# burn-research/OpenMEASURE

Measured on AMD Instinct MI355X. Metric: SPR fit+reconstruct throughput (GB/s snapshot matrix), higher is better.
Workload: dtype f64

## Files before the change

### include/spr_hip.h

```cpp
#ifndef SPR_HIP_H
#define SPR_HIP_H

#include <stddef.h>
#include <stdint.h>

#ifdef __cplusplus
extern "C" {
#endif

#define SPR_OK 0
#define SPR_E_INVALID (-1)
#define SPR_E_UNSUPPORTED (-2)
#define SPR_E_HIP (-3)
#define SPR_E_WORKSPACE (-4)

#define SPR_MAX_M 256
#define SPR_MAX_M_WIDE 512
#define SPR_MAX_R 128
#define SPR_MAX_R_STREAM 256
#define SPR_MAX_R_WIDE 1024

#define SPR_ABI_VERSION 5
int spr_abi_version(void);
const char *spr_last_error(void);
// ... 68 lines not shown
int spr_project_stream_norms_f64(const double *d_X, int64_t n_rows, int32_t m, int64_t ldx, int64_t row0,
                                 int64_t n_points, int32_t n_features, int32_t center, const double *d_inv_scale,
                                 const double *d_rowmean, const double *d_W, int32_t r, double *d_Ur, int64_t ldu,
                                 double *d_rownorm2, void *d_workspace, size_t workspace_bytes, void *stream);

int spr_scale_rows_f64(const double *d_X, int64_t n_rows, int32_t m, int64_t ldx, int64_t row0,
                       int64_t n_points, int32_t n_features, const double *d_rowmean,
                       const double *d_inv_scale, double *d_X0, int64_t ldo, void *stream);
int spr_unscale_f64(const double *d_x0, int64_t n_rows, int64_t row0, int64_t n_points,
                    int32_t n_features, const double *d_rowmean, const double *d_scale,
                    const double *d_rowscale, double *d_x, void *stream);

size_t spr_feature_minmax_workspace(int32_t n_features);
int spr_feature_minmax_f64(const double *d_X, int64_t n_rows, int32_t m, int64_t ldx, int64_t row0,
                           int64_t n_points, int32_t n_features, double *d_minmax,
                           void *d_workspace, size_t workspace_bytes, void *stream);

int spr_feature_digit_hist_f64(const double *d_X, int64_t n_rows, int32_t m, int64_t ldx, int64_t row0,
                               int64_t n_points, int32_t n_features, const uint64_t *d_prefix, int32_t shift,
                               int32_t bits, int32_t two_targets, uint64_t *d_hist, void *stream);

size_t spr_colsums_workspace(int32_t m, int32_t n_features);
int spr_colsums_f64(const double *d_X, int64_t n_rows, int32_t m, int64_t ldx, int64_t row0,
                    int64_t n_points, int32_t n_features, const double *d_rowmean, double *d_out,
                    void *d_workspace, size_t workspace_bytes, void *stream);
int spr_fill_feature_f64(double *d_out, int64_t n_rows, int64_t row0, int64_t n_points, int32_t n_features,
                         const double *d_values, void *stream);

int spr_reconstruct_f64(const double *d_Ur, int64_t n_rows, int32_t r, int64_t ldu,
                        int64_t row0, int64_t n_points, int32_t n_features,
                        const double *d_rowmean, const double *d_scale, const double *d_rowscale,
                        const double *d_A, int32_t n_p, double *d_Xrec, int64_t ldo,
                        void *stream);
size_t spr_bound_sweep_workspace(int32_t n_p, int32_t n_features);
int spr_bound_sweep_f64(const double *d_Ur, int64_t n_rows, int32_t r, int64_t ldu, int64_t row0, int64_t n_points,
                        int32_t n_features, const double *d_rowmean, const double *d_scale, const double *d_limits,
                        const double *d_clamp, const double *d_G, int32_t n_p, double tol, int32_t k, double *d_out,
                        void *d_workspace, size_t workspace_bytes, void *stream);
int spr_bound_sweep_u32(const float *d_Ur, int64_t n_rows, int32_t r, int64_t ldu, int64_t row0, int64_t n_points,
                        int32_t n_features, const double *d_rowmean, const double *d_scale, const double *d_limits,
                        const double *d_clamp, const double *d_G, int32_t n_p, double tol, int32_t k, double *d_out,
                        void *d_workspace, size_t workspace_bytes, void *stream);
size_t spr_bound_sweep_batch_workspace(int32_t n_p, int32_t n_features);
int spr_bound_sweep_batch_f64(const double *d_Ur, int64_t n_rows, int32_t r, int64_t ldu, int64_t row0, int64_t n_points,
                              int32_t n_features, const double *d_rowmean, const double *d_scale, const double *d_limits,
                              const double *d_clamp, const double *d_G, int32_t n_p, double tol, int32_t k, double *d_out,
                              void *d_workspace, size_t workspace_bytes, void *stream);
int spr_bound_sweep_batch_u32(const float *d_Ur, int64_t n_rows, int32_t r, int64_t ldu, int64_t row0, int64_t n_points,
                              int32_t n_features, const double *d_rowmean, const double *d_scale, const double *d_limits,
                              const double *d_clamp, const double *d_G, int32_t n_p, double tol, int32_t k, double *d_out,
                              void *d_workspace, size_t workspace_bytes, void *stream);
size_t spr_encode_workspace(int32_t r, int32_t k, int32_t n_features);
int spr_encode_f64(const double *d_Ur, int64_t n_rows, int32_t r, int64_t ldu, const double *d_X, int32_t k, int64_t ldx,
                   int64_t row0, int64_t n_points, int32_t n_features, const double *d_rowmean, const double *d_scale,
                   double *d_A, void *d_workspace, size_t workspace_bytes, void *stream);
int spr_encode_x32(const double *d_Ur, int64_t n_rows, int32_t r, int64_t ldu, const float *d_X, int32_t k, int64_t ldx,
                   int64_t row0, int64_t n_points, int32_t n_features, const double *d_rowmean, const double *d_scale,
                   double *d_A, void *d_workspace, size_t workspace_bytes, void *stream);
int spr_encode_u32(const float *d_Ur, int64_t n_rows, int32_t r, int64_t ldu, const double *d_X, int32_t k, int64_t ldx,
                   int64_t row0, int64_t n_points, int32_t n_features, const double *d_rowmean, const double *d_scale,
                   double *d_A, void *d_workspace, size_t workspace_bytes, void *stream);
int spr_encode_x32_u32(const float *d_Ur, int64_t n_rows, int32_t r, int64_t ldu, const float *d_X, int32_t k, int64_t ldx,
                       int64_t row0, int64_t n_points, int32_t n_features, const double *d_rowmean, const double *d_scale,
                       double *d_A, void *d_workspace, size_t workspace_bytes, void *stream);
size_t spr_field_error_workspace(int32_t k, int32_t n_features);
int spr_field_error_f64(const double *d_Ur, int64_t n_rows, int32_t r, int64_t ldu, int64_t row0, int64_t n_points,
// ... 311 lines not shown
```

### openmeasure_amd/_lib.py

```python
from __future__ import annotations

import ctypes as C
import os

_HERE = os.path.dirname(os.path.abspath(__file__))
LIB_PATH = os.environ.get('SPR_HIP_LIBRARY') or os.path.join(_HERE, 'libspr_hip.so')

SPR_ABI_VERSION = 5
SPR_MAX_M = 256
SPR_MAX_M_WIDE = 512
SPR_MAX_R = 128
SPR_MAX_R_STREAM = 256
SPR_MAX_R_WIDE = 1024
SPR_GP_MAX_M = 800
SPR_GP_MAX_D = 8

_i32, _i64, _u64, _sz = C.c_int32, C.c_int64, C.c_uint64, C.c_size_t
_p = C.c_void_p
_dbl = C.c_double

PROTOTYPES = {
    'spr_abi_version': (C.c_int, []),
    'spr_last_error': (C.c_char_p, []),
    'spr_device_cus': (C.c_int, [C.POINTER(C.c_int)]),
# ... 1 lines not shown
    'spr_download_bytes': (C.c_int, [_p, _p, _i64, _p, _u64, _p]),
    'spr_host_tridiag_vectors': (C.c_int, [_p, _p, _i32, _p, _i32, _p, _i32]),
    'spr_host_eig_top': (C.c_int, [_p, _i32, _i32, _p, _p, _p, _p, _p]),
    'spr_host_svd_top': (C.c_int, [_p, _i32, _i32, _p, _p, _p, _p, _p]),
    'spr_stats_gram_workspace': (_sz, [_i32, _i32]),
    'spr_stats_gram_f64': (C.c_int, [_p, _i64, _i32, _i64, _i64, _i64, _i32, _i32, _p, _p, _sz, _p]),
    'spr_stats_gram_finalize_f64': (C.c_int, [_i64, _i32, _i64, _i64, _i32, _p, _sz, _p, _p, _i32, _i32, _p]),
    'spr_stats_gram_shifted_f64': (C.c_int, [_p, _i64, _i32, _i64, _i64, _i64, _i32, _p, _p, _p, _sz, _p]),
    'spr_gram_shift_finish_f64': (C.c_int, [_p, _p, _i64, _i32, _i32, _p, _i32, _p]),
    'spr_rowstats_workspace': (_sz, [_i32]),
    'spr_rowstats_f64': (C.c_int, [_p, _i64, _i32, _i64, _i64, _i64, _i32, _p, _p, _p, _sz, _p]),
    'spr_gram_cross_workspace': (_sz, [_i32, _i32]),
    'spr_gram_cross_f64': (C.c_int, [_p, _i64, _i32, _i64, _i64, _i64, _i32, _i32, _p, _p, _p, _sz, _p]),
    'spr_gram_cross_pair_f64': (C.c_int, [_p, _i64, _i32, _i32, _i32, _i32, _i64, _i64, _i64, _i32, _i32, _p, _p, _p, _sz, _p]),
    'spr_rowmean_stats_f64': (C.c_int, [_p, _i64, _i64, _i64, _i32, _p, _p, _sz, _p]),
    'spr_spectrum_max_m': (_i32, []),
    'spr_spectrum_f64': (C.c_int, [_p, _p, _i32, _i32, _i32, _i32, _i32, _p, _p, _p, _p, _p, _p, _p, _p, _p, _p, _p]),
    'spr_gram_combine_f64': (C.c_int, [_p, _p, _i32, _i32, _i32, _i32, _p, _p, _p, _p, _p]),
    'spr_project_f64': (C.c_int, [_p, _i64, _i32, _i64, _i64, _i64, _i32, _i32, _p, _p, _p, _i32, _p, _i64, _i32, _p]),
    'spr_project_norms_supported': (_i32, [_i32, _i32, _i64, _i64, _p, _i32]),
    'spr_project_norms_f64': (C.c_int, [_p, _i64, _i32, _i64, _i64, _i64, _i32, _i32, _p, _p, _p, _i32, _p, _i64, _p, _p]),
    'spr_project_stream_norms_f64': (C.c_int, [_p, _i64, _i32, _i64, _i64, _i64, _i32, _i32, _p, _p, _p, _i32, _p, _i64, _p, _p, _sz, _p]),
    'spr_project_stream_workspace': (_sz, [_i32, _i32, _i32]),
    'spr_project_stream_f64': (C.c_int, [_p, _i64, _i32, _i64, _i64, _i64, _i32, _i32, _p, _p, _p, _i32, _p, _i64, _p, _sz, _p]),
    'spr_scale_rows_f64': (C.c_int, [_p, _i64, _i32, _i64, _i64, _i64, _i32, _p, _p, _p, _i64, _p]),
    'spr_unscale_f64': (C.c_int, [_p, _i64, _i64, _i64, _i32, _p, _p, _p, _p, _p]),
    'spr_feature_minmax_workspace': (_sz, [_i32]),
    'spr_feature_minmax_f64': (C.c_int, [_p, _i64, _i32, _i64, _i64, _i64, _i32, _p, _p, _sz, _p]),
    'spr_feature_digit_hist_f64': (C.c_int, [_p, _i64, _i32, _i64, _i64, _i64, _i32, _p, _i32, _i32, _i32, _p, _p]),
    'spr_colsums_workspace': (_sz, [_i32, _i32]),
    'spr_colsums_f64': (C.c_int, [_p, _i64, _i32, _i64, _i64, _i64, _i32, _p, _p, _p, _sz, _p]),
    'spr_fill_feature_f64': (C.c_int, [_p, _i64, _i64, _i64, _i32, _p, _p]),
    'spr_reconstruct_f64': (C.c_int, [_p, _i64, _i32, _i64, _i64, _i64, _i32, _p, _p, _p, _p, _i32, _p, _i64, _p]),
    'spr_bound_sweep_workspace': (_sz, [_i32, _i32]),
    'spr_bound_sweep_f64': (C.c_int, [_p, _i64, _i32, _i64, _i64, _i64, _i32, _p, _p, _p, _p, _p, _i32, _dbl, _i32, _p, _p, _sz, _p]),
    'spr_bound_sweep_batch_workspace': (_sz, [_i32, _i32]),
    'spr_bound_sweep_batch_f64': (C.c_int, [_p, _i64, _i32, _i64, _i64, _i64, _i32, _p, _p, _p, _p, _p, _i32, _dbl, _i32, _p, _p, _sz, _p]),
    'spr_encode_workspace': (_sz, [_i32, _i32, _i32]),
    'spr_encode_f64': (C.c_int, [_p, _i64, _i32, _i64, _p, _i32, _i64, _i64, _i64, _i32, _p, _p, _p, _p, _sz, _p]),
    'spr_field_error_workspace': (_sz, [_i32, _i32]),
    'spr_field_error_f64': (C.c_int, [_p, _i64, _i32, _i64, _i64, _i64, _i32, _p, _p, _p, _i32, _p, _i64, _p, _p, _sz, _p]),
    'spr_gappy_normal_workspace': (_sz, [_i32, _i32, _i32]),
    'spr_gappy_normal_f64': (C.c_int, [_p, _i64, _i32, _i64, _p, _i32, _i64, _i64, _i64, _i32, _p, _p, _p, _i64, _p, _p, _p, _p, _sz, _p]),
    'spr_gappy_fill_workspace': (_sz, []),
    'spr_gappy_rowfill_f64': (C.c_int, [_p, _i64, _i32, _i64, _i64, _p, _i64, _p, _p, _sz, _p]),
    'spr_gappy_fill_f64': (C.c_int, [_p, _i64, _i32, _i64, _p, _i32, _i64, _i64, _i64, _i32, _p, _p, _p, _p, _i64, _p, _p, _sz, _p]),
    'spr_field_std_diag_f64': (C.c_int, [_p, _i64, _i32, _i64, _i64, _i64, _i32, _p, _p, _p, _i32, _p, _i64, _p]),
    'spr_field_std_factor_f64': (C.c_int, [_p, _i64, _i32, _i64, _i64, _i64, _i32, _p, _p, _p, _i32, _i32, _p, _i64, _p]),
    'spr_gp_workspace': (_sz, [_i32, _i32]),
    'spr_gp_train_f64': (C.c_int, [_p, _i32, _i32, _i64, _p, _i32, _i64, _i32, _p, _dbl, _i32, _dbl, _p, _p, _p, _p, _p, _sz, _p]),
    'spr_gp_predict_f64': (C.c_int, [_p, _i32, _i32, _i64, _p, _i32, _i64, _i32, _p, _i32, _p, _p, _p, _p, _p]),
    'spr_gp_workspace_ard': (_sz, [_i32, _i32, _i32]),
    'spr_gp_train_ard_f64': (C.c_int, [_p, _i32, _i32, _i64, _p, _i32, _i64, _i32, _i32, _p, _dbl, _i32, _dbl, _p, _p, _p, _p, _p, _sz, _p]),
    'spr_gp_predict_ard_f64': (C.c_int, [_p, _i32, _i32, _i64, _p, _i32, _i64, _i32, _i32, _p, _i32, _p, _p, _p, _p, _p]),
    'spr_field_unstage_f64': (C.c_int, [_p, _i32, _i32, _i64, _p, _i64, _p]),
    'spr_field_unstage_blocks_f64': (C.c_int, [_p, _i32, _i32, _i64, _p, _p, _i64, _p]),
    'spr_p2p_handle_bytes': (_sz, []),
    'spr_p2p_alloc': (C.c_int, [_sz, _i32, _p, _p]),
    'spr_p2p_free': (C.c_int, [_p]),
    'spr_p2p_open': (C.c_int, [_p, _p]),
    'spr_p2p_close': (C.c_int, [_p]),
    'spr_p2p_device_id': (C.c_int, [_p, _i32]),
    'spr_p2p_peer_access': (C.c_int, [_p, _p]),
    'spr_p2p_signal': (C.c_int, [_p, _u64, _p]),
    'spr_p2p_wait': (C.c_int, [_p, _u64, _p]),
    'spr_p2p_flags_set': (C.c_int, [_p, _i32, _u64, _p]),
# ... 36 lines not shown
    'spr_allreduce_f64': (C.c_int, [_p, _p, _i64, _p]),
    'spr_allreduce_i64': (C.c_int, [_p, _p, _i64, _p]),
    'spr_allgather': (C.c_int, [_p, _p, _p, _i64, _p]),
    'spr_fit_gram_pass_buffer': (_sz, [_i32, _i32, _i32]),
    'spr_fit_gram_pass_workspace': (_sz, [_i32, _i32, _i64]),
    'spr_fit_gram_pass': (C.c_int, [_p, _p, _i32, _i64, _i32, _i64, _i64, _i64, _i32, _i32, _p, _p, _sz, _p, _p, _p, _p, _p, _sz, _p]),
    'spr_synth_f64': (C.c_int, [_p, _i64, _i32, _i64, _i64, _i64, _i32, _p, _i32, _i32, _dbl, _u64, _p]),
    'spr_synth_gather_f64': (C.c_int, [_p, _i32, _i64, _i32, _p, _i32, _i32, _dbl, _u64, _p, _p]),
}

_lib = None


class SprError(RuntimeError):
    """A libspr_hip.so call returned a negative status."""


PROTOTYPES['spr_project_x32_acc'] = (C.c_int, [_p, _i64, _i32, _i64, _i64, _i64, _i32, _i32, _p, _p, _p, _i32, _p, _i64, _p, _i64, _p])

for _f64, _x32 in (('spr_stats_gram_f64', 'spr_stats_gram_x32'), ('spr_stats_gram_shifted_f64', 'spr_stats_gram_shifted_x32'), ('spr_rowstats_f64', 'spr_rowstats_x32'),
                   ('spr_gram_cross_f64', 'spr_gram_cross_x32'), ('spr_gram_cross_pair_f64', 'spr_gram_cross_pair_x32'), ('spr_project_f64', 'spr_project_x32'),
                   ('spr_project_f64', 'spr_project_x32_f64out'),
                   ('spr_project_stream_f64', 'spr_project_stream_x32'),
                   ('spr_project_stream_f64', 'spr_project_stream_x32_f64out'),
                   ('spr_project_norms_f64', 'spr_project_norms_x32'),
                   ('spr_project_norms_f64', 'spr_project_norms_x32_f64out'),
                   ('spr_project_stream_norms_f64', 'spr_project_stream_norms_x32'),
                   ('spr_project_stream_norms_f64', 'spr_project_stream_norms_x32_f64out'),
                   ('spr_qr_init_norms_f64', 'spr_qr_init_norms_u32'),
                   ('spr_qr_epoch_sweep_f64', 'spr_qr_epoch_sweep_u32'),
                   ('spr_scale_rows_f64', 'spr_scale_rows_x32'), ('spr_feature_minmax_f64', 'spr_feature_minmax_x32'),
                   ('spr_colsums_f64', 'spr_colsums_x32'), ('spr_feature_digit_hist_f64', 'spr_feature_digit_hist_x32'),
                   ('spr_synth_f64', 'spr_synth_f32'), ('spr_reconstruct_f64', 'spr_reconstruct_u32'),
                   ('spr_bound_sweep_f64', 'spr_bound_sweep_u32'),
                   ('spr_bound_sweep_batch_f64', 'spr_bound_sweep_batch_u32'),
                   ('spr_encode_f64', 'spr_encode_x32'), ('spr_encode_f64', 'spr_encode_u32'),
                   ('spr_encode_f64', 'spr_encode_x32_u32'),
                   ('spr_field_error_f64', 'spr_field_error_x32'), ('spr_field_error_f64', 'spr_field_error_u32'),
                   ('spr_field_error_f64', 'spr_field_error_x32_u32'),
                   ('spr_gappy_normal_f64', 'spr_gappy_normal_x32'), ('spr_gappy_normal_f64', 'spr_gappy_normal_u32'),
                   ('spr_gappy_normal_f64', 'spr_gappy_normal_x32_u32'),
                   ('spr_gappy_rowfill_f64', 'spr_gappy_rowfill_x32'),
                   ('spr_gappy_fill_f64', 'spr_gappy_fill_x32'), ('spr_gappy_fill_f64', 'spr_gappy_fill_u32'),
                   ('spr_gappy_fill_f64', 'spr_gappy_fill_x32_u32'),
                   ('spr_field_std_diag_f64', 'spr_field_std_diag_u32'),
                   ('spr_field_std_factor_f64', 'spr_field_std_factor_u32'),
                   ('spr_mask_rows_f64', 'spr_mask_rows_u32'), ('spr_qr_init_f64', 'spr_qr_init_u32'),
                   ('spr_qr_refresh_f64', 'spr_qr_refresh_u32'), ('spr_measure_csr_f64', 'spr_measure_csr_u32')):
    PROTOTYPES[_x32] = PROTOTYPES[_f64]


def load():
    global _lib
    if _lib is not None:
        return _lib
    if not os.path.exists(LIB_PATH):
        raise RuntimeError(
            f'{LIB_PATH} is missing: build it with `make -C openmeasure_amd/csrc` '
            '(or __graft_entry__.build()). There is no CPU fallback for the SPR kernels.')
    import torch
    lib = C.CDLL(LIB_PATH, mode=C.RTLD_GLOBAL)
    for name, (res, args) in PROTOTYPES.items():
        fn = getattr(lib, name)
        fn.restype = res
        fn.argtypes = args
    have = lib.spr_abi_version()
# ... 14 lines not shown
```

### openmeasure_amd/_shard.py

```python
from __future__ import annotations

import numpy as np

class RowShard:

    def __init__(self, row0, n_global, group=None, force_collectives=False, broadcast_basis=False, partial=False,
                 gather='auto', native_comm=False):
        if gather not in ('auto', 'p2p', 'rccl'):
            raise ValueError("gather must be 'auto', 'p2p' or 'rccl'")
        self.native_comm = bool(native_comm)
        self.row0 = int(row0)
        self.n_global = int(n_global)
        self.group = group
        self.force_collectives = bool(force_collectives)
        self.broadcast_basis = bool(broadcast_basis)
        self.partial = bool(partial)
        self.gather = gather

    @property
    def world(self):
        import torch.distributed as dist
        return dist.get_world_size(self.group) if dist.is_available() and dist.is_initialized() else 1

    @property
    def rank(self):
        import torch.distributed as dist
        return dist.get_rank(self.group) if dist.is_available() and dist.is_initialized() else 0


class PendingField:

    def __init__(self, tensor, works=(), keep=(), on_wait=None, join=None, needs_cus=True, launch=None, shape=None):
        self._tensor = tensor
        self._works = list(works)
        self._join = join
        self._keep = keep
        self._on_wait = on_wait
        self._launch = launch
        self._inner = None
        self._shape = tuple(shape) if shape is not None else None
        self._needs_cus = bool(needs_cus)

    @property
    def needs_cus(self):
        if self._inner is not None:
            return self._inner.needs_cus
        return self._needs_cus and (bool(self._works) or self._join is not None)

    @property
    def shape(self):
        return self._shape if self._tensor is None else tuple(self._tensor.shape)

    @property
    def launched(self):
        return self._launch is None

    @property
    def pending(self):
        if self._launch is not None:
            return True
        if self._inner is not None:
            return self._inner.pending
        return bool(self._works) or self._join is not None

    def launch(self):
        fn, self._launch = self._launch, None
        if fn is not None:
            res = fn()
            if isinstance(res, PendingField):
                self._inner = res
            else:
                self._tensor = res

    def wait(self):
        self.launch()
        if self._inner is not None:
            self._tensor = self._inner.wait()
            self._inner = None
            return self._tensor
        done = self._on_wait() if ((self._works or self._join is not None) and self._on_wait is not None) else None
        for w in self._works:
            w.wait()
        if self._join is not None:
            self._join()
        if done is not None:
            done()
        self._works = []
        self._join = None
        self._keep = ()
        self._on_wait = None
        return self._tensor


class ShardedOps:

    def _world(self):
        return self._shard.world if self._shard is not None else 1

    def _dist(self):
        return self._shard is not None and (self._shard.world > 1 or self._shard.force_collectives)

    def _shard_layout(self, n_loc):
        lay = self.__dict__.get('_layout')
        if lay is None:
            eng = self._engine()
            src = self.__dict__.pop('_layout_src', None)
            if src is not None:
                rows = np.rint(eng.to_host(src[0].sum(1))).astype(np.int64)
# ... 398 lines not shown
```

### openmeasure_amd/csrc/reconstruct.hip

```cpp
#include <stdlib.h>

#include <type_traits>

#include "rowtile.hpp"
#include "launch.hpp"

#ifndef SPR_RECONSTRUCT_VALU
#define SPR_RECONSTRUCT_VALU 0
#endif

namespace {

constexpr int RM_THREADS = 256;
constexpr int RM_PB = 16;

template <int MTR, int VEC, typename TU>
__global__ __launch_bounds__(RM_THREADS) void reconstruct_mfma_kernel(
    const TU *__restrict__ Ur, int r, int64_t ldu, SegPlan plan, const double *__restrict__ rowmean,
    const double *__restrict__ scale, const double *__restrict__ rowscale, const double *__restrict__ A, int64_t lda,
    int np0, int npb, double *__restrict__ out, int64_t ldo, int accumulate) {
  constexpr int NW = RM_THREADS / 64, R = 64;
  constexpr int MPAD = 16 * MTR, MP = MPAD + 2, KSTEPS = MPAD / 4;
  using RT = RowTile<MTR, R, MP, NW, 16, TU>;
  __shared__ double smem[2 * R * MP];
// ... 276 lines not shown
  SPR_REQUIRE_LAYOUT(name, row0, n_rows, n_points, n_features);
  hipStream_t st = static_cast<hipStream_t>(stream);
  if (!std::is_same<TU, double>::value || !SPR_RECONSTRUCT_VALU || r > SPR_MAX_R)
    return reconstruct_groups<TU>(d_Ur, n_rows, r, ldu, row0, n_points, n_features, d_rowmean, d_scale, d_rowscale, d_A, n_p,
                                  d_Xrec, ldo, st);
  if constexpr (std::is_same<TU, double>::value) {
    const int half = (r + 1) / 2;
#define RC(L) return launch<L>(d_Ur, n_rows, r, ldu, row0, n_points, n_features, d_rowmean, d_scale, d_rowscale, d_A, n_p, d_Xrec, ldo, st)
    if (half <= 1) RC(1);
    if (half <= 2) RC(2);
    if (half <= 4) RC(4);
    if (half <= 8) RC(8);
    if (half <= 16) RC(16);
    if (half <= 32) RC(32);
    RC(64);
#undef RC
  }
  return SPR_E_UNSUPPORTED;
}
}

#define SPR_RECONSTRUCT_ENTRY(NAME, TU)                                                                                       \
  SPR_ENTRY(NAME,                                                                                                             \
            (const TU *d_Ur, int64_t n_rows, int32_t r, int64_t ldu, int64_t row0, int64_t n_points, int32_t n_features,      \
             const double *d_rowmean, const double *d_scale, const double *d_rowscale, const double *d_A, int32_t n_p,        \
             double *d_Xrec, int64_t ldo, void *stream),                                                                      \
            (reconstruct<TU>), d_Ur, n_rows, r, ldu, row0, n_points, n_features, d_rowmean, d_scale, d_rowscale, d_A, n_p,    \
            d_Xrec, ldo, stream)
SPR_RECONSTRUCT_ENTRY(spr_reconstruct_f64, double)
SPR_RECONSTRUCT_ENTRY(spr_reconstruct_u32, float)
#undef SPR_RECONSTRUCT_ENTRY

namespace {
__global__ __launch_bounds__(256) void field_unstage_kernel(const double *__restrict__ stage, int world, int n_p,
                                                            int64_t n_loc, double *__restrict__ out, int64_t ldo) {
  const int q = blockIdx.y / n_p, v = blockIdx.y - q * n_p;
  const double *src = stage + ((int64_t)q * n_p + v) * n_loc;
  double *dst = out + (int64_t)v * ldo + (int64_t)q * n_loc;
  const bool vec = ((reinterpret_cast<uintptr_t>(src) | reinterpret_cast<uintptr_t>(dst)) & 15) == 0;
  const int64_t stride = (int64_t)gridDim.x * 256;
  if (vec) {
    const int64_t n2 = n_loc / 2;
    for (int64_t i = (int64_t)blockIdx.x * 256 + threadIdx.x; i < n2; i += stride)
      reinterpret_cast<f64x2 *>(dst)[i] = __builtin_nontemporal_load(reinterpret_cast<const f64x2 *>(src) + i);
    if ((n_loc & 1) && blockIdx.x == 0 && threadIdx.x == 0) dst[n_loc - 1] = src[n_loc - 1];
  } else {
    for (int64_t i = (int64_t)blockIdx.x * 256 + threadIdx.x; i < n_loc; i += stride) dst[i] = src[i];
  }
}
}

extern "C" int spr_field_unstage_f64(const double *d_stage, int32_t world, int32_t n_p, int64_t n_loc, double *d_out,
                                     int64_t ldo, void *stream) {
  SPR_REQUIRE(d_stage && d_out, SPR_E_INVALID, "spr_field_unstage_f64: NULL pointer");
  SPR_REQUIRE(world > 0 && n_p > 0 && n_loc > 0 && ldo >= (int64_t)world * n_loc && (int64_t)world * n_p <= 65535,
              SPR_E_INVALID, "spr_field_unstage_f64: bad shape world=%d n_p=%d n_loc=%lld ldo=%lld", world, n_p,
              (long long)n_loc, (long long)ldo);
  int64_t bx = (n_loc / 2 + 255) / 256;
  if (bx > 1024) bx = 1024;
  if (bx < 1) bx = 1;
  hipLaunchKernelGGL(field_unstage_kernel, dim3((unsigned)bx, (unsigned)(world * n_p)), dim3(256), 0,
                     static_cast<hipStream_t>(stream), d_stage, (int)world, (int)n_p, n_loc, d_out, ldo);
  SPR_LAUNCH_CHECK();
  return SPR_OK;
}

// ... 36 lines not shown
```

### openmeasure_amd/engine.py

```python
from __future__ import annotations

import numpy as np

from . import _lib


def _ptr(t):
    return t.data_ptr() if t is not None else None


_NP_OF = {'torch.float64': np.float64, 'torch.float32': np.float32, 'torch.int64': np.int64, 'torch.int32': np.int32,
          'torch.uint8': np.uint8, 'torch.int8': np.int8, 'torch.int16': np.int16, 'torch.bool': np.bool_}


class HipEngine:
    name = 'hip-gfx950'

    supports_row_norms = True
    supports_gram_out = True

    def __init__(self, device=None):
        import torch
        self.torch = torch
        if not torch.cuda.is_available():
            raise RuntimeError('openmeasure_amd needs an AMD GPU visible to PyTorch-ROCm; '
                               'there is no CPU fallback for the SPR kernels.')
        self.lib = _lib.load()
        self.device = torch.device(device if device is not None else f'cuda:{torch.cuda.current_device()}')
        self._ws = {}
        self._timing = {}
        import os
        self._force_stream = os.environ.get('SPR_PROJECT_STREAM') == '1'
        self._dl_kernel = os.environ.get('SPR_DL_KERNEL', '1') != '0'
        self._stage = None
        import atexit
        import weakref
        ref = weakref.ref(self)
        atexit.register(lambda: ref() is not None and ref().close(wait=False))

    def close(self, wait=True):
        torch = self.torch
        if wait:
            try:
                torch.cuda.synchronize(self.device)
            except RuntimeError:
                pass
        pool = self.__dict__.pop('_copy_pool', None)
        if pool is not None:
            pool.shutdown(wait=wait, cancel_futures=not wait)
        self._stage = None
        for k in ('_dstage2', '_dstage_slots', '_dl', '_reuse', '_side'):
            self.__dict__.pop(k, None)
        try:
            torch._C._host_emptyCache()
        except (AttributeError, RuntimeError):
            pass

    def _stream(self):
        return self.torch.cuda.current_stream(self.device).cuda_stream

    def empty(self, shape, dtype=None):
        return self.torch.empty(shape, dtype=dtype or self.torch.float64, device=self.device)

    def zeros(self, shape, dtype=None):
        return self.torch.zeros(shape, dtype=dtype or self.torch.float64, device=self.device)

    _STAGE_BYTES = 1 << 20
    _STAGE_SLOTS = 8

    def to_device(self, a, dtype=None):
        torch = self.torch
        if dtype is None:
            dtype = torch.float64
        t = torch.as_tensor(np.ascontiguousarray(a))
        if t.dtype != dtype:
            t = t.to(dtype)
        nbytes = t.numel() * t.element_size()
        if nbytes == 0 or nbytes > self._STAGE_BYTES or nbytes % 8:
            return t.to(device=self.device).contiguous()
        if self._stage is None:
            self._stage = [[torch.empty(self._STAGE_BYTES, dtype=torch.uint8, pin_memory=True), None]
                           for _ in range(self._STAGE_SLOTS)]
            self._stage_next = 0
        slot = self._stage[self._stage_next]
# ... 614 lines not shown
                   _ptr(ws), ws.numel(), self._stream())
        return out

    def fill_feature(self, n_rows, row0, n_points, values):
        out = self.empty((n_rows,))
        self._call(self.lib.spr_fill_feature_f64, _ptr(out), n_rows, row0, n_points, values.shape[0], _ptr(values),
                   self._stream())
        return out

    def scale_rows(self, X, row0, n_points, n_features, rowmean, inv_scale):
        n, m, ld = self._check_matrix(X)
        out = self.empty((n, m))
        self._call(self._x('spr_scale_rows', X), _ptr(X), n, m, ld, row0, n_points, n_features, _ptr(rowmean),
                   _ptr(inv_scale), _ptr(out), m, self._stream())
        return out

    def unscale(self, x0, row0, n_points, n_features, rowmean, scale, rowscale=None):
        n = x0.shape[0]
        out = self.empty((n,))
        self._call(self.lib.spr_unscale_f64, _ptr(x0.contiguous()), n, row0, n_points, n_features, _ptr(rowmean),
                   _ptr(scale), _ptr(rowscale), _ptr(out), self._stream())
        return out

    def reconstruct(self, Ur, row0, n_points, n_features, rowmean, scale, A, out=None, rowscale=None):
        n, r, ldu = self._check_matrix(Ur)
        n_p = A.shape[0]
        if out is None:
            out = self.empty((n_p, n))
        self._call(self._u('spr_reconstruct', Ur), _ptr(Ur), n, r, ldu, row0, n_points, n_features, _ptr(rowmean),
                   _ptr(scale), _ptr(rowscale), _ptr(A.contiguous()), n_p, _ptr(out), out.stride(0), self._stream(),
                   timed='reconstruct')
        return out

    def bound_sweep(self, Ur, row0, n_points, n_features, rowmean, scale, limits, clamp, G, tol, k):
        n, r, ldu = self._check_matrix(Ur)
        n_p = G.shape[0]
        out = self.empty((n_p, 3 + 3 * k))
        ws = self._workspace('bound_sweep', self.lib.spr_bound_sweep_workspace(n_p, n_features))
        self._call(self._u('spr_bound_sweep', Ur), _ptr(Ur), n, r, ldu, row0, n_points, n_features, _ptr(rowmean),
                   _ptr(scale), _ptr(limits.contiguous()), _ptr(clamp.contiguous()), _ptr(G.contiguous()), n_p, float(tol),
                   int(k), _ptr(out), _ptr(ws), ws.numel(), self._stream(), timed='bound_sweep')
        return out

    def bound_sweep_batch(self, Ur, row0, n_points, n_features, rowmean, scale, limits, clamp, G, tol, k):
        n, r, ldu = self._check_matrix(Ur)
        n_p = G.shape[0]
        out = self.empty((n_p, 3 + 3 * k))
        ws = self._workspace('bound_sweep', self.lib.spr_bound_sweep_batch_workspace(n_p, n_features))
        self._call(self._u('spr_bound_sweep_batch', Ur), _ptr(Ur), n, r, ldu, row0, n_points, n_features, _ptr(rowmean),
                   _ptr(scale), _ptr(limits.contiguous()), _ptr(clamp.contiguous()), _ptr(G.contiguous()), n_p, float(tol),
                   int(k), _ptr(out), _ptr(ws), ws.numel(), self._stream(), timed='bound_sweep_batch')
        return out

    def _ux(self, base, Ur, X):
        t = self.torch
        x32, u32 = X.dtype == t.float32, Ur.dtype == t.float32
        return getattr(self.lib, base + ('_x32_u32' if x32 and u32 else '_x32' if x32 else '_u32' if u32 else '_f64'))

    def _check_columns(self, Ur, X):
        n, r, ldu = self._check_matrix(Ur)
        if isinstance(X, self.torch.Tensor) and X.dim() == 2 and X.shape[1] == 1 and X.stride(1) != 1:
            X = X.as_strided(X.shape, (X.stride(0), 1))
        nx, k, ldx = self._check_matrix(X)
        if nx != n:
            raise ValueError(f'the matrix has {nx} rows, the basis block {n}')
        return X, n, r, ldu, k, ldx
# ... 407 lines not shown
```

### openmeasure_amd/rom.py

```python
from __future__ import annotations

from collections import namedtuple

import numpy as np

from . import _eigen
from ._lib import SPR_MAX_R, SPR_MAX_R_WIDE
from ._placement import GemPlacement, _check_mask, pivot_loop
from ._shard import PendingField, RowShard, ShardedOps

__all__ = ['ROM', 'SPR', 'RowShard', 'DeviceMatrix', 'PendingField', 'OneHotRows']

_DEVICE_SPECTRUM_MAX_M = 24
_GRAM_KAPPA_REFINE = 1e4
_GRAM_REFINE_MAX_PASSES = 3
_DENSE_C_LIMIT = 1 << 26


class DeviceMatrix:

    def __init__(self, tensor, basis=None):
        if basis not in (None, 'f64', 'f32'):
            raise ValueError("basis must be None / 'f64' / 'f32'")
        self.tensor = tensor
# ... 161 lines not shown

class _DeviceState(dict):

    def __init__(self, stash=None, upload=None):
        super().__init__()
        self.stash = dict(stash or {})
        self.upload = upload

    def __missing__(self, key):
        if key in self.stash:
            t = self[key] = self.upload(self.stash.pop(key))
            return t
        raise KeyError(key)

    def __contains__(self, key):
        return dict.__contains__(self, key) or key in self.stash

    def get(self, key, default=None):
        try:
            return self[key]
        except KeyError:
            return default

    def pop(self, key, *default):
        if not dict.__contains__(self, key) and key in self.stash:
            del self.stash[key]
            if default:
                return default[0]
            raise KeyError(key)
        return dict.pop(self, key, *default)


_TRANSIENT = ('_eng', '_d', '_trace', '_pending', '_pending_field', '_gram_events', '_gram_events_pending', '_layout_src',
              '_gap_t0', '_G', '_last_decomp', 'comm_timing', 'last_comm_', '_layout', '_p2p', '_gather_sel', '_basis_checked', '_basis_diverged', '_deferred', '_row0_d', '_ncomm', '_combined', '_comm_stream')


class ROM(ShardedOps):

    def __init__(self, X, n_features, xyz, shard=None, engine=None):
        if isinstance(X, DeviceMatrix):
            pass
        elif type(X) is not np.ndarray:
            raise TypeError('The matrix X is not a numpy array.')
        if type(n_features) is not int:
            raise TypeError('The parameter n_features is not an integer.')
        self.X = X
        self.n_features = n_features
        self.xyz = xyz
        self._shard = shard
        n = shard.n_global if shard is not None else X.shape[0]
        self.n_points = n // self.n_features
        if n % self.n_features != 0:
            raise Exception('The number of rows of X is not a multiple of n_features')
        self._n_global = n
        self._row0 = shard.row0 if shard is not None else 0
        if self._row0 + X.shape[0] > n:
            raise ValueError('The local row block does not fit in the global matrix.')
        self._eng = engine
        self._d = _DeviceState()
        self._host = {}

    cpod_tol = 1e-9
    cpod_rows_per_round = 64
    cpod_max_rounds = 60
    cpod_max_rows = 4000

    def CPOD(self, problem_dict, **kwargs):
# ... 42 lines not shown
        d_host = dict(self._d.stash)
        for k, t in self._d.items():
            if k == 'X' and not isinstance(self.X, DeviceMatrix):
                continue
            d_host[k] = eng.to_host(t)
        if isinstance(self.X, DeviceMatrix):
            state['X'] = d_host.pop('X') if 'X' in d_host else eng.to_host(self.X.tensor)
            state['_basis_f32'] = self.X.basis == 'f32'
        state['_d_host'] = d_host
        if self._shard is not None:
            sh = RowShard(self._shard.row0, self._shard.n_global, None, self._shard.force_collectives,
                          self._shard.broadcast_basis, self._shard.partial, self._shard.gather, self._shard.native_comm)
            state['_shard'] = sh
        return state

    def __setstate__(self, state):
        d_host = state.pop('_d_host', {})
        self.__dict__.update(state)
        self._eng = None

        def upload(a):
            eng = self._engine()
            return eng.to_device(a, dtype=eng.torch.float32 if a.dtype == np.float32 else None)
        self._d = _DeviceState(d_host, upload)

    _LAZY = ('Ar', 'Sigma_r', 'Vr', 'exp_variance_', 'S_', '_scl_f', '_var_f')

    placement_norms = False

    gap_filler = False

    defer_reconstruct = True

    def _flush_deferred(self):
        pf = self.__dict__.pop('_deferred', None)
        if pf is not None and not pf.launched:
            pf.launch()
            return True
        return False
    _GAP_FILL_FRACTION = 0.85
    _GAP_FILL_MIN_M = 128
    _GAP_FILL_MIN_MS = 2.2

    comm_timing = None

    def _comm_bracket(self, key):
        ct = self.comm_timing
        eng = self._engine()
        if ct is None or not hasattr(eng, 'timing_event'):
            return lambda: None
        e0 = eng.timing_event()

        def close():
            ct.setdefault(key, []).append((e0, eng.timing_event()))
        return close

    def __getattr__(self, name):
        pend = self.__dict__.get('_pending')
        if pend is not None and name in ROM._LAZY:
            self._materialize()
            if name in self.__dict__:
                return self.__dict__[name]
        raise AttributeError(f"'{type(self).__name__}' object has no attribute '{name}'")

    def _materialize(self):
        pend = self.__dict__.pop('_pending', None)
        if pend is None:
            return
        eng = self._engine()
        r = pend['r']
        feat = eng.to_host(pend['feat'])
        S = eng.to_host(pend['S'])
# ... 700 lines not shown
            m = X0d.shape[1]
            S, V, exp_variance = self._spectrum(G, lambda ev: self._select_rank(ev, m, select_modes, n_modes))
            r = self._select_rank(exp_variance, m, select_modes, n_modes)
            floor = S[0] * np.sqrt(m * np.finfo(float).eps)
            if S[r - 1] * _GRAM_KAPPA_REFINE < S[0]:
                S, V, exp_variance, _ = self._refine_spectrum(S, V, r, X0d, 0, X0d.shape[0], 1, ones, None, False,
                                                              rank_of=lambda ev: self._select_rank(ev, m, select_modes, n_modes))
                r = self._select_rank(exp_variance, m, select_modes, n_modes)
                floor = S[0] * m * np.finfo(float).eps
            W = V[:, :r] / np.maximum(S[:r], floor if floor > 0 else 1.0)
            Ur_d = eng.project(X0d, 0, X0d.shape[0], 1, ones, eng.to_device(W), center=False)
            Ar, expv = V[:, :r] * S[:r], exp_variance[:r]
        self.r = r
        Ur = np.ascontiguousarray(eng.to_host(Ur_d))
        self._last_decomp = (Ur, Ur_d)
        return Ur, Ar, expv

    def fit(self, scale_type='std', axis_cnt=1, select_modes='variance', n_modes=99, basis=None):
        axis_cnt = self._check_scaling(scale_type, axis_cnt)
        if basis is None and select_modes not in ('variance', 'number'):
            raise ValueError('The select_mode value is wrong.')
        eng = self._engine()
        self.scale_type = scale_type
        for k in ROM._LAZY + ('C', 'Theta', '_pending', '_cpod_Ar0'):
            self.__dict__.pop(k, None)
        if basis is not None:
            self._basis_foreign = 'fit(basis=...) took the basis from the caller'
        elif str(self._basis_dtype()) == 'torch.float32':
            self._basis_foreign = "DeviceMatrix(basis='f32') stores the basis in float32: orthonormal to f32 rounding only"
        else:
            self._basis_foreign = None
        for k in ('cnt', 'Theta', 'nrm0'):
            self._d.pop(k, None)
        took = self._device_fit(scale_type, axis_cnt, select_modes, n_modes, basis)
        if took is True:
            return
        if took != 'merged':
            self._fit_fills_gap = basis is None
            try:
                self._stats_pass(scale_type, axis_cnt)
            finally:
                self._fit_fills_gap = False
        self._host.clear()
        if basis is None:
            Ur_d, Ar, expv, S, r, V_r = self._basis_from_gram(self._G, select_modes, n_modes, True, self._d['inv_scale'])
            self.exp_variance_ = expv
            self.S_ = S
        else:
            self._flush_deferred()
            Ur_d = eng.to_device(basis[0])
            Ar = np.asarray(basis[1])
            V_r = None
        self._d['Ur'] = Ur_d
        if '_layout_src' in self.__dict__ and '_layout' not in self.__dict__:
            self._shard_layout(Ur_d.shape[0])
        self.Ar = Ar
        self.r = Ar.shape[1]
        Sigma_r = np.linalg.norm(Ar, axis=0)
        self.Sigma_r = Sigma_r
        if V_r is not None:
            self.Vr = V_r * (np.linalg.norm(V_r, axis=0) ** -1)
        else:
            self.Vr = Ar / Sigma_r
        self._trace.report()

    def _device_fit(self, scale_type, axis_cnt, select_modes, n_modes, basis):
# ... 28 lines not shown
        feat = chk[5:].reshape(F, 5)
        self._scl_f, self._mu_f = feat[:, 3].copy(), feat[:, 1].copy()
        self._set_precenter_ratio(feat[:, 1], feat[:, 2], feat[:, 4], axis_cnt)
        good = bool(np.all(np.isfinite(chk)))
        if good:
            converged = chk[2] < eng.spectrum_max_sweeps or chk[3] <= 1e-24 * chk[4]
            kappa = chk[0] / chk[1] if chk[1] > 0 else np.inf
            good = converged and not kappa > _GRAM_KAPPA_REFINE and not self._needs_precenter(kappa)
        if not good:
            self._merge_stats(gram, fs_all, rowmean, scale_type, axis_cnt)
            self._device_fit_fallback_ = True
            return 'merged'
        self.r = r
        self.gram_refine_passes_ = 0
        self.precentered_ = False
        sp['r'] = r
        self._pending = sp
        tr_.report()
        return True

    def reconstruct(self, Ar, sampling=None, to_host=True, wait=True):
        eng = self._engine()
        self._flush_deferred()
        defer = sampling is None and self._defers() and not to_host and not wait
        A_d = self._coefficients(eng, Ar, own=defer)
        if A_d.shape[0] == 0:
            rows = self._n_global if sampling is None else sampling.shape[0]
            return np.zeros((rows, 0)) if to_host else eng.empty((0, rows))
        if sampling is not None:
            Th, cnt, scl = self._sampled(sampling)
            ones = eng.to_device(np.ones(1))
            Thp = Th if Th.shape[1] % 2 == 0 else eng.torch.nn.functional.pad(Th, (0, 1))[:, :Th.shape[1]]
            out = eng.reconstruct(Thp, 0, Th.shape[0], 1, cnt, ones, A_d, rowscale=scl)
            return out if not to_host else eng.to_host(out, result=True).T
        state = self._block()
        if defer:
            n_loc, n_p = state.Ur.shape[0], A_d.shape[0]
            total = int(self._shard_layout(n_loc)[:, 1].sum()) if self._dist() else n_loc
            pf = self._deferred = PendingField(None, launch=lambda: self._reconstruct_now(A_d, state, False, False),
                                               shape=(n_p, total), needs_cus=False)
            return pf
        return self._reconstruct_now(A_d, state, to_host, wait)

    def _defers(self):
        import os
        env = os.environ.get('SPR_DEFER_RECONSTRUCT')
        return (self.defer_reconstruct or env == '1') and env != '0'

    def _reconstruct_now(self, A_d, state, to_host, wait, path=None):
        eng = self._engine()
        n_loc = state.Ur.shape[0]
        n_p = A_d.shape[0]
        world = self._world()
        if not self._dist():
            if to_host and hasattr(eng, 'reconstruct_to_host'):
                host = eng.reconstruct_to_host(*state, A_d)
                if host is not None:
                    return host.T
            out = eng.reconstruct(*state, A_d)
        else:
            import torch.distributed as dist
            lay = self._shard_layout(n_loc)
            if (path or self._gather_select(n_p, lay)) == 'p2p':
                return self._reconstruct_p2p(A_d, state, lay, to_host, wait)
            if np.any(lay[:, 1] != n_loc):
                return self._gather_unequal(A_d, state, lay, to_host, wait)
            loc = eng.reconstruct(*state, A_d)
            stage = eng.empty((world, n_p, n_loc))
            close = self._comm_bracket('gather')
            import time
            self.last_comm_ = ('field all_gather (rccl)', (world, n_p, n_loc), time.time())
            nc = self._native_comm()
            if nc is not None:
                t = eng.torch
                side = self.__dict__.get('_comm_stream')
                if side is None:
                    side = self._comm_stream = t.cuda.Stream(eng.device)
                ev0 = t.cuda.Event()
                ev0.record(t.cuda.current_stream(eng.device))
                side.wait_event(ev0)
                with t.cuda.stream(side):
                    eng.comm_allgather(nc, loc, stage)
                    ev1 = t.cuda.Event()
                    ev1.record(side)
                loc.record_stream(side)
                stage.record_stream(side)
# ... 646 lines not shown
```

Measured before the change: 1175.

## Overlap deferred single-vector reconstruct with next fit's Gram on side stream

Adds a dedicated wave-per-16-rows reconstruct kernel for a single coefficient vector, with software-pipelined register prefetch of basis pieces. When a deferred reconstruct is still pending as the next fit starts, the kernel is launched on a separate HIP stream ordered by events, so it runs concurrently with the fit's Gram and stats passes. This is meant to hide reconstruct time behind the bandwidth-heavy fit. The cost is extra stream and event bookkeeping, contention for memory bandwidth and CUs between the two kernels, and reliance on record_stream and event waits to keep results correct.

```diff
diff --git a/include/spr_hip.h b/include/spr_hip.h
--- a/include/spr_hip.h
+++ b/include/spr_hip.h
@@ -124,6 +124,12 @@
                         const double *d_rowmean, const double *d_scale, const double *d_rowscale,
                         const double *d_A, int32_t n_p, double *d_Xrec, int64_t ldo,
                         void *stream);
+int spr_reconstruct_guest_f64(const double *d_Ur, int64_t n_rows, int32_t r, int64_t ldu, int64_t row0, int64_t n_points,
+                              int32_t n_features, const double *d_rowmean, const double *d_scale, const double *d_a,
+                              double *d_xrec, void *stream);
+int spr_reconstruct_guest_u32(const float *d_Ur, int64_t n_rows, int32_t r, int64_t ldu, int64_t row0, int64_t n_points,
+                              int32_t n_features, const double *d_rowmean, const double *d_scale, const double *d_a,
+                              double *d_xrec, void *stream);
 size_t spr_bound_sweep_workspace(int32_t n_p, int32_t n_features);
 int spr_bound_sweep_f64(const double *d_Ur, int64_t n_rows, int32_t r, int64_t ldu, int64_t row0, int64_t n_points,
                         int32_t n_features, const double *d_rowmean, const double *d_scale, const double *d_limits,
diff --git a/openmeasure_amd/_lib.py b/openmeasure_amd/_lib.py
--- a/openmeasure_amd/_lib.py
+++ b/openmeasure_amd/_lib.py
@@ -57,6 +57,7 @@
     'spr_colsums_f64': (C.c_int, [_p, _i64, _i32, _i64, _i64, _i64, _i32, _p, _p, _p, _sz, _p]),
     'spr_fill_feature_f64': (C.c_int, [_p, _i64, _i64, _i64, _i32, _p, _p]),
     'spr_reconstruct_f64': (C.c_int, [_p, _i64, _i32, _i64, _i64, _i64, _i32, _p, _p, _p, _p, _i32, _p, _i64, _p]),
+    'spr_reconstruct_guest_f64': (C.c_int, [_p, _i64, _i32, _i64, _i64, _i64, _i32, _p, _p, _p, _p, _p]),
     'spr_bound_sweep_workspace': (_sz, [_i32, _i32]),
     'spr_bound_sweep_f64': (C.c_int, [_p, _i64, _i32, _i64, _i64, _i64, _i32, _p, _p, _p, _p, _p, _i32, _dbl, _i32, _p, _p, _sz, _p]),
     'spr_bound_sweep_batch_workspace': (_sz, [_i32, _i32]),
@@ -159,6 +160,7 @@
                    ('spr_scale_rows_f64', 'spr_scale_rows_x32'), ('spr_feature_minmax_f64', 'spr_feature_minmax_x32'),
                    ('spr_colsums_f64', 'spr_colsums_x32'), ('spr_feature_digit_hist_f64', 'spr_feature_digit_hist_x32'),
                    ('spr_synth_f64', 'spr_synth_f32'), ('spr_reconstruct_f64', 'spr_reconstruct_u32'),
+                   ('spr_reconstruct_guest_f64', 'spr_reconstruct_guest_u32'),
                    ('spr_bound_sweep_f64', 'spr_bound_sweep_u32'),
                    ('spr_bound_sweep_batch_f64', 'spr_bound_sweep_batch_u32'),
                    ('spr_encode_f64', 'spr_encode_x32'), ('spr_encode_f64', 'spr_encode_u32'),
diff --git a/openmeasure_amd/_shard.py b/openmeasure_amd/_shard.py
--- a/openmeasure_amd/_shard.py
+++ b/openmeasure_amd/_shard.py
@@ -37,6 +37,8 @@
         self._keep = keep
         self._on_wait = on_wait
         self._launch = launch
+        self._event = None
+        self.path = None
         self._inner = None
         self._shape = tuple(shape) if shape is not None else None
         self._needs_cus = bool(needs_cus)
@@ -63,17 +65,24 @@
             return self._inner.pending
         return bool(self._works) or self._join is not None
 
-    def launch(self):
-        fn, self._launch = self._launch, None
-        if fn is not None:
-            res = fn()
+    def launch(self, fn=None):
+        rec, self._launch = self._launch, None
+        if rec is not None:
+            res = (fn or rec)()
             if isinstance(res, PendingField):
                 self._inner = res
+            elif isinstance(res, tuple):
+                self._tensor, self._event, self._keep = res
             else:
                 self._tensor = res
 
+    def order(self):
+        if self._event is not None:
+            self._event.wait()
+
     def wait(self):
         self.launch()
+        self.order()
         if self._inner is not None:
             self._tensor = self._inner.wait()
             self._inner = None
diff --git a/openmeasure_amd/csrc/reconstruct.hip b/openmeasure_amd/csrc/reconstruct.hip
--- a/openmeasure_amd/csrc/reconstruct.hip
+++ b/openmeasure_amd/csrc/reconstruct.hip
@@ -332,6 +332,180 @@
 #undef SPR_RECONSTRUCT_ENTRY
 
 namespace {
+constexpr int RL_THREADS = 256;
+
+template <bool VEC, bool FULL, typename TU>
+__global__ __launch_bounds__(RL_THREADS) __attribute__((amdgpu_waves_per_eu(8, 8))) void reconstruct_guest_kernel(
+    const TU *__restrict__ Ur, int64_t n_rows, int r, int64_t ldu, int64_t row0, int64_t n_points,
+    const double *__restrict__ rowmean, const double *__restrict__ scale, const double *__restrict__ a,
+    double *__restrict__ out) {
+  constexpr int PW = 2, CW = 8 * PW;
+  typedef TU Piece __attribute__((ext_vector_type(PW)));
+  typedef double Coef __attribute__((ext_vector_type(PW)));
+  const int lane = threadIdx.x & 63;
+  const int jj = lane >> 3, c = lane & 7;
+  const int np = (r + 2 * CW - 1) / (2 * CW);
+  const int64_t nfull = n_rows / 16;
+  const int64_t nwave = (int64_t)gridDim.x * (RL_THREADS / 64);
+  int64_t b = (int64_t)blockIdx.x * (RL_THREADS / 64) + __builtin_amdgcn_readfirstlane(threadIdx.x >> 6);
+  if (16 * b >= n_rows) return;
+  const unsigned lo = (unsigned)jj * (unsigned)ldu + PW * c;
+  auto load = [&](const TU *base, int g) {
+    Piece v;
+    if (FULL) {
+      v = *reinterpret_cast<const Piece *>(base + lo);
+    } else {
+      const int col = CW * g + PW * c;
+      const TU *rp = base + (unsigned)jj * (unsigned)ldu - CW * g;
+      if (VEC) {
+        v = *reinterpret_cast<const Piece *>(rp + (col < r ? col : 0));
+      } else {
+#pragma unroll
+        for (int t = 0; t < PW; ++t) v[t] = rp[col + t < r ? col + t : 0];
+      }
+    }
+    return v;
+  };
+  auto coef = [&](int g) {
+    const int col = CW * g + PW * c;
+    Coef v;
+    if (FULL) {
+      v = *reinterpret_cast<const Coef *>(a + col);
+    } else if (VEC) {
+      v = *reinterpret_cast<const Coef *>(a + (col < r ? col : 0));
+    } else {
+#pragma unroll
+      for (int t = 0; t < PW; ++t) v[t] = a[col + t < r ? col + t : 0];
+    }
+    return v;
+  };
+  auto dot_piece = [&](const Piece &v, const Coef &cf, int g, double d) {
+#pragma unroll
+    for (int t = 0; t < PW; ++t) {
+      if (FULL) {
+        d += (double)v[t] * cf[t];
+      } else {
+        const bool in = CW * g + PW * c + t < r;
+        d += (in ? (double)v[t] : 0.0) * (in ? cf[t] : 0.0);
+      }
+    }
+    return d;
+  };
+  auto row_terms = [&](int64_t blk, int &f, int64_t &fend, double &mu, double &sc) {
+    if (16 * blk >= fend) {
+      f = (int)((row0 + 16 * blk) / n_points);
+      fend = (int64_t)(f + 1) * n_points - row0;
+    }
+    const int64_t row = 16 * blk + 8 * (c & 1) + jj;
+    const int64_t rc = row < n_rows ? row : n_rows - 1;
+    int fr = f + (rc >= fend ? 1 : 0);
+    if (n_points < 16)
+      fr = f + (int)(rc - (fend - n_points)) / (int)n_points;
+    mu = rowmean[rc];
+    sc = scale[fr];
+  };
+  auto finish = [&](double d0, double d1, double mu, double sc, int64_t blk) {
+    d0 = group_sum_t<8>(d0);
+    d1 = group_sum_t<8>(d1);
+    const double dot = (c & 1) ? d1 : d0;
+    const int64_t row = 16 * blk + 8 * (c & 1) + jj;
+    if (c < 2 && row < n_rows) out[row] = sc * dot + mu;
+  };
+  if (b == 0 && 16 * nfull < n_rows) {
+    int f = (int)((row0 + 16 * nfull) / n_points);
+    int64_t fend = (int64_t)(f + 1) * n_points - row0;
+    double mu, sc;
+    row_terms(nfull, f, fend, mu, sc);
+    double d0 = 0.0, d1 = 0.0;
+    auto row_elem = [&](int q, int k) {
+      const int64_t rq = 16 * nfull + 8 * q + jj;
+      return (double)Ur[(rq < n_rows ? rq : n_rows - 1) * ldu + k];
+    };
+#pragma unroll 1
+    for (int k0 = PW * c; k0 < r; k0 += CW)
+#pragma unroll
+      for (int t = 0; t < PW; ++t)
+        if (k0 + t < r) {
+          d0 += row_elem(0, k0 + t) * a[k0 + t];
+          d1 += row_elem(1, k0 + t) * a[k0 + t];
+        }
+    finish(d0, d1, mu, sc, nfull);
+  }
+  if (b < nfull) {
+    int f = (int)((row0 + 16 * b) / n_points);
+    int64_t fend = (int64_t)(f + 1) * n_points - row0;
+    const int64_t hstep = 8 * ldu, bstep = 16 * nwave * ldu;
+    const TU *pn = Ur + 16 * b * ldu;
+    Piece u0 = load(pn, 0), u1 = load(pn + hstep, 0), u2 = load(pn + CW, 1), u3 = load(pn + hstep + CW, 1);
+    Coef nA = coef(0), nB = coef(1);
+    while (b < nfull) {
+      const int64_t bn = b + nwave;
+      double mu, sc;
+      row_terms(b, f, fend, mu, sc);
+      double d0 = 0.0, d1 = 0.0;
+#pragma unroll 1
+      for (int p = 0; p < np; ++p) {
+        const bool last = p + 1 == np;
+        const int pq = last ? 0 : p + 1;
+        if (last && bn < nfull) pn += bstep;
+        const TU *pu = pn + 2 * CW * pq;
+        const Coef cA = nA, cB = nB;
+        nA = coef(2 * pq);
+        nB = coef(2 * pq + 1);
+        d0 = dot_piece(u0, cA, 2 * p, d0);
+        u0 = load(pu, 2 * pq);
+        __builtin_amdgcn_sched_barrier(0);
+        d1 = dot_piece(u1, cA, 2 * p, d1);
+        u1 = load(pu + hstep, 2 * pq);
+        __builtin_amdgcn_sched_barrier(0);
+        d0 = dot_piece(u2, cB, 2 * p + 1, d0);
+        u2 = load(pu + CW, 2 * pq + 1);
+        __builtin_amdgcn_sched_barrier(0);
+        d1 = dot_piece(u3, cB, 2 * p + 1, d1);
+        u3 = load(pu + hstep + CW, 2 * pq + 1);
+        __builtin_amdgcn_sched_barrier(0);
+      }
+      finish(d0, d1, mu, sc, b);
+      b = bn;
+    }
+  }
+}
+
+template <typename TU>
+int reconstruct_guest(const char *name, const TU *d_Ur, int64_t n_rows, int32_t r, int64_t ldu, int64_t row0,
+                      int64_t n_points, int32_t n_features, const double *d_rowmean, const double *d_scale,
+                      const double *d_a, double *d_xrec, void *stream) {
+  SPR_REQUIRE(d_Ur && d_rowmean && d_scale && d_a && d_xrec, SPR_E_INVALID, "%s: NULL pointer", name);
+  SPR_REQUIRE(n_rows > 0 && r > 0 && ldu >= r, SPR_E_INVALID, "%s: bad shape n_rows=%lld r=%d ldu=%lld", name,
+              (long long)n_rows, r, (long long)ldu);
+  SPR_REQUIRE_LAYOUT(name, row0, n_rows, n_points, n_features);
+  SPR_REQUIRE(r <= SPR_MAX_R, SPR_E_UNSUPPORTED, "%s: r = %d exceeds %d", name, r, SPR_MAX_R);
+  hipStream_t st = static_cast<hipStream_t>(stream);
+  const int grid = spr_cus_or_default();
+  SPR_REQUIRE(ldu < ((int64_t)1 << 24), SPR_E_UNSUPPORTED, "%s: row stride %lld too long", name, (long long)ldu);
+  const bool vec = spr_pair_aligned(d_Ur, r, ldu) && (reinterpret_cast<uintptr_t>(d_a) & 15) == 0;
+  const bool full = vec && r % 32 == 0;
+#define RL(V, F_) hipLaunchKernelGGL((reconstruct_guest_kernel<V, F_, TU>), dim3(grid), dim3(RL_THREADS), 0, st, d_Ur, n_rows, \
+                                     (int)r, ldu, row0, n_points, d_rowmean, d_scale, d_a, d_xrec)
+  if (full) RL(true, true);
+  else if (vec) RL(true, false);
+  else RL(false, false);
+#undef RL
+  SPR_LAUNCH_CHECK();
+  return SPR_OK;
+}
+}
+
+SPR_ENTRY(spr_reconstruct_guest_f64,
+          (const double *d_Ur, int64_t n_rows, int32_t r, int64_t ldu, int64_t row0, int64_t n_points, int32_t n_features,
+           const double *d_rowmean, const double *d_scale, const double *d_a, double *d_xrec, void *stream),
+          (reconstruct_guest<double>), d_Ur, n_rows, r, ldu, row0, n_points, n_features, d_rowmean, d_scale, d_a, d_xrec, stream)
+SPR_ENTRY(spr_reconstruct_guest_u32,
+          (const float *d_Ur, int64_t n_rows, int32_t r, int64_t ldu, int64_t row0, int64_t n_points, int32_t n_features,
+           const double *d_rowmean, const double *d_scale, const double *d_a, double *d_xrec, void *stream),
+          (reconstruct_guest<float>), d_Ur, n_rows, r, ldu, row0, n_points, n_features, d_rowmean, d_scale, d_a, d_xrec, stream)
+
+namespace {
 __global__ __launch_bounds__(256) void field_unstage_kernel(const double *__restrict__ stage, int world, int n_p,
                                                             int64_t n_loc, double *__restrict__ out, int64_t ldo) {
   const int q = blockIdx.y / n_p, v = blockIdx.y - q * n_p;
diff --git a/openmeasure_amd/engine.py b/openmeasure_amd/engine.py
--- a/openmeasure_amd/engine.py
+++ b/openmeasure_amd/engine.py
@@ -49,7 +49,7 @@
         if pool is not None:
             pool.shutdown(wait=wait, cancel_futures=not wait)
         self._stage = None
-        for k in ('_dstage2', '_dstage_slots', '_dl', '_reuse', '_side'):
+        for k in ('_dstage2', '_dstage_slots', '_dl', '_reuse', '_side', '_guest_stream'):
             self.__dict__.pop(k, None)
         try:
             torch._C._host_emptyCache()
@@ -730,6 +730,32 @@
                    timed='reconstruct')
         return out
 
+    def stream_event(self):
+        ev = self.torch.cuda.Event()
+        ev.record(self.torch.cuda.current_stream(self.device))
+        return ev
+
+    def reconstruct_guest_takes(self, Ur, rowmean, A):
+        return (A.shape[0] == 1 and 0 < Ur.shape[1] <= _lib.SPR_MAX_R and rowmean.shape[0] == Ur.shape[0]
+                and Ur.stride(1) == 1)
+
+    def reconstruct_guest(self, Ur, row0, n_points, n_features, rowmean, scale, A):
+        torch = self.torch
+        n, r, ldu = self._check_matrix(Ur)
+        side = self.__dict__.get('_guest_stream')
+        if side is None:
+            side = self._guest_stream = torch.cuda.Stream(self.device)
+        A = A.contiguous()
+        out = self.empty((1, n))
+        side.wait_event(self.stream_event())
+        with torch.cuda.stream(side):
+            self._call(self._u('spr_reconstruct_guest', Ur), _ptr(Ur), n, r, ldu, row0, n_points, n_features, _ptr(rowmean),
+                       _ptr(scale), _ptr(A), _ptr(out), self._stream(), timed='reconstruct')
+            done = self.stream_event()
+        for t in (Ur, rowmean, scale, A, out):
+            t.record_stream(side)
+        return out, done
+
     def bound_sweep(self, Ur, row0, n_points, n_features, rowmean, scale, limits, clamp, G, tol, k):
         n, r, ldu = self._check_matrix(Ur)
         n_p = G.shape[0]
diff --git a/openmeasure_amd/rom.py b/openmeasure_amd/rom.py
--- a/openmeasure_amd/rom.py
+++ b/openmeasure_amd/rom.py
@@ -217,7 +217,7 @@
 
 
 _TRANSIENT = ('_eng', '_d', '_trace', '_pending', '_pending_field', '_gram_events', '_gram_events_pending', '_layout_src',
-              '_gap_t0', '_G', '_last_decomp', 'comm_timing', 'last_comm_', '_layout', '_p2p', '_gather_sel', '_basis_checked', '_basis_diverged', '_deferred', '_row0_d', '_ncomm', '_combined', '_comm_stream')
+              '_gap_t0', '_G', '_last_decomp', 'comm_timing', 'last_comm_', '_layout', '_p2p', '_gather_sel', '_basis_checked', '_basis_diverged', '_deferred', '_guest_pending', '_row0_d', '_ncomm', '_combined', '_comm_stream')
 
 
 class ROM(ShardedOps):
@@ -326,12 +326,47 @@
 
     defer_reconstruct = True
 
-    def _flush_deferred(self):
+    reconstruct_under_gram = True
+
+    reconstruct_path_ = None
+
+    def _flush_deferred(self, under_gram=None):
+        if under_gram is None:
+            self._join_guest()
         pf = self.__dict__.pop('_deferred', None)
         if pf is not None and not pf.launched:
-            pf.launch()
+            fn = None
+            if under_gram is not None:
+                fn = self._guest_launch(pf, under_gram)
+                if fn is None:
+                    self._deferred = pf
+                    return False
+                self._guest_pending = pf
+            pf.launch(fn)
             return True
         return False
+
+    def _join_guest(self):
+        pf = self.__dict__.pop('_guest_pending', None)
+        if pf is not None:
+            pf.order()
+
+    def _guest_launch(self, pf, Xd):
+        import os
+        env = os.environ.get('SPR_RECONSTRUCT_GUEST')
+        eng = self._engine()
+        args = getattr(pf, 'deferred_args', None)
+        if not ((self.reconstruct_under_gram or env == '1') and env != '0') or args is None or self._dist():
+            return None
+        A_d, state = args
+        if not hasattr(eng, 'reconstruct_guest') or Xd.shape[1] > 256 or not eng.reconstruct_guest_takes(state.Ur, state.rowmean, A_d):
+            return None
+
+        def launch():
+            out, done = eng.reconstruct_guest(*state, A_d)
+            self.reconstruct_path_ = pf.path = 'guest'
+            return out, done, (state, A_d)
+        return launch
     _GAP_FILL_FRACTION = 0.85
     _GAP_FILL_MIN_M = 128
     _GAP_FILL_MIN_MS = 2.2
@@ -1098,6 +1133,7 @@
             self._basis_foreign = None
         for k in ('cnt', 'Theta', 'nrm0'):
             self._d.pop(k, None)
+        self._flush_deferred(under_gram=self._Xd())
         took = self._device_fit(scale_type, axis_cnt, select_modes, n_modes, basis)
         if took is True:
             return
@@ -1192,13 +1228,20 @@
             ones = eng.to_device(np.ones(1))
             Thp = Th if Th.shape[1] % 2 == 0 else eng.torch.nn.functional.pad(Th, (0, 1))[:, :Th.shape[1]]
             out = eng.reconstruct(Thp, 0, Th.shape[0], 1, cnt, ones, A_d, rowscale=scl)
+            self.reconstruct_path_ = 'stream'
             return out if not to_host else eng.to_host(out, result=True).T
         state = self._block()
         if defer:
             n_loc, n_p = state.Ur.shape[0], A_d.shape[0]
             total = int(self._shard_layout(n_loc)[:, 1].sum()) if self._dist() else n_loc
-            pf = self._deferred = PendingField(None, launch=lambda: self._reconstruct_now(A_d, state, False, False),
-                                               shape=(n_p, total), needs_cus=False)
+            def launch():
+                if self._dist():
+                    return self._reconstruct_now(A_d, state, False, False)
+                out = self._reconstruct_now(A_d, state, False, True)
+                pf.path = self.reconstruct_path_
+                return (out, eng.stream_event(), ()) if hasattr(eng, 'stream_event') else out
+            pf = self._deferred = PendingField(None, launch=launch, shape=(n_p, total), needs_cus=False)
+            pf.deferred_args = (A_d, state)
             return pf
         return self._reconstruct_now(A_d, state, to_host, wait)
 
@@ -1212,6 +1255,7 @@
         n_loc = state.Ur.shape[0]
         n_p = A_d.shape[0]
         world = self._world()
+        self.reconstruct_path_ = 'stream'
         if not self._dist():
             if to_host and hasattr(eng, 'reconstruct_to_host'):
                 host = eng.reconstruct_to_host(*state, A_d)
```

Result: no change. 1179, median of 3 (+0.4%).
